# MarToonLi/StableDiffusionEO

Measured on AMD Instinct MI355X. Metric: 512x512 canny2image images/sec (20 DDIM steps); ms per UNet step reported alongside, higher is better.
Workload: dtype f16; 1 GPU; SD1.5 + ControlNet-canny 512x512, batch=1 per GPU (CFG pair fused, N=2), 20 DDIM steps + VAE decode, fp16 storage / fp32 accumulate (BASELINE configs[1]); model_config=sd15, ddim_steps=20, parallelism=dp1 (image index -> rank, RCCL all_gather of final latents), weights=seeded synthetic (no checkpoint in the container)

## Files before the change

stablediffusioneo_amd/csrc/api_ops.hip:

```cpp
#include <stdarg.h>

#include "../../include/sdeo.h"
#include "sdeo_internal.h"
#include "kernels.h"

namespace sdeo {

static thread_local std::string g_last_error;

void set_error(const std::string& msg) { g_last_error = msg; }

int fail(const char* fmt, ...) {
  char buf[1024];
  va_list ap;
  va_start(ap, fmt);
  vsnprintf(buf, sizeof(buf), fmt, ap);
  va_end(ap);
  g_last_error = buf;
  return 1;
}

}

using namespace sdeo;
// ... 253 lines not shown
}

int sdeo_debug_gemm_stats_f16(void* y, int ldy, const void* x, int ldx, const void* w, int ldw, const float* bias, const void* res,
                              int ldres, int m, int n, int k, float* stats, int stats_ld, int* strips_out, void* stream) {
  SDEO_CHECK(stats && strips_out, "gemm_stats: null argument");
  ConvGemm p;
  fill_gemm(p, m, n, k);
  p.x = (const f16*)x; p.w = (const f16*)w; p.bias = bias; p.res = (const f16*)res; p.y = (f16*)y;
  p.ldx = ldx; p.ldw = ldw; p.ldy = ldy; p.ldres = ldres;
  *strips_out = conv_gemm_stats_strips(p);
  if (*strips_out == 0) return 0;
  SDEO_CHECK(*strips_out <= stats_ld, "gemm_stats: %d strips do not fit stats_ld %d", *strips_out, stats_ld);
  p.stats_out = stats; p.stats_ld = stats_ld;
  return conv_gemm(p, S(stream));
}

int sdeo_debug_gemm_res_rows_f16(void* y, int ldy, const void* x, int ldx, const void* w, int ldw, const float* bias, const void* res,
                                 int ldres, int res_rows, int m, int n, int k, float* stats, int stats_ld, int* strips_out, void* workspace,
                                 size_t workspace_bytes, void* stream) {
  ConvGemm p;
  fill_gemm(p, m, n, k);
  p.x = (const f16*)x; p.w = (const f16*)w; p.bias = bias; p.res = (const f16*)res; p.y = (f16*)y;
  p.ldx = ldx; p.ldw = ldw; p.ldy = ldy; p.ldres = ldres; p.res_rows = res_rows;
  p.workspace = (float*)workspace; p.workspace_bytes = workspace_bytes;
  if (stats) {
    SDEO_CHECK(strips_out, "gemm_res_rows: null argument");
    *strips_out = conv_gemm_stats_strips(p);
    SDEO_CHECK(*strips_out <= stats_ld, "gemm_res_rows: %d strips do not fit stats_ld %d", *strips_out, stats_ld);
    if (*strips_out > 0) { p.stats_out = stats; p.stats_ld = stats_ld; }
  }
  return conv_gemm(p, S(stream));
}

int sdeo_debug_gemm_ln_f16(void* y, int ldy, const void* x, int ldx, const void* w_folded, int ldw, const float* ln_s,
                           const float* bias_folded, const float* stats, int stats_ld, int strips, int ln_c, int m, int n, int k, int act, float eps, void* workspace, size_t workspace_bytes, void* stream) {
  ConvGemm p;
  fill_gemm(p, m, n, k);
  p.x = (const f16*)x; p.w = (const f16*)w_folded; p.bias = bias_folded; p.y = (f16*)y;
  p.ldx = ldx; p.ldw = ldw; p.ldy = ldy; p.act = act;
  p.ln_stats = stats; p.ln_s = ln_s; p.ln_strips = strips; p.ln_ld = stats_ld; p.ln_c = ln_c; p.ln_eps = eps;
  p.workspace = (float*)workspace; p.workspace_bytes = workspace_bytes;
  return conv_gemm(p, S(stream));
}

int sdeo_debug_row_stats_f16(float* stats, int stats_ld, const void* x, int ldx, int rows, int c, void* stream) {
  return row_stats(stats, stats_ld, (const f16*)x, ldx, rows, c, S(stream));
}

int sdeo_layernorm_f16(void* y, const void* x, const float* gamma, const float* beta, int rows, int c, float eps,
                       void* stream) {
  return layernorm((f16*)y, c, (const f16*)x, c, gamma, beta, rows, c, eps, S(stream));
}

int sdeo_debug_layernorm_ld_f16(void* y, int ldy, const void* x, int ldx, const float* gamma, const float* beta, int rows, int c,
                                float eps, void* stream) {
  SDEO_CHECK(ldx >= c && ldy >= c, "layernorm_ld: ldx=%d ldy=%d below c=%d", ldx, ldy, c);
  return layernorm((f16*)y, ldy, (const f16*)x, ldx, gamma, beta, rows, c, eps, S(stream));
}

int sdeo_debug_softmax_rows(void* p, int ldp, const float* s, int lds, int rows, int cols, float scale, void* stream) {
  SDEO_CHECK(ldp >= cols && lds >= cols, "softmax_rows: ldp=%d lds=%d below cols=%d", ldp, lds, cols);
  return softmax_rows((f16*)p, ldp, s, lds, rows, cols, scale, S(stream));
}

int sdeo_attention_f16(void* o, int ldo, const void* q, int ldq, const void* k, int ldk, const void* v, int ldv, int b,
                       int heads, int tq, int tk, int tk_stride, int vt_batch_stride, int d, float scale, void* stream) {
// ... 59 lines not shown
```

stablediffusioneo_amd/csrc/conv_gemm.hip:

```cpp
#include <stdlib.h>

#include <array>
#include <map>

#include <type_traits>
#include <utility>

#include "conv_inl.h"

namespace sdeo {

template <int BM, int BN, int STAGES, bool UPS, bool WS, bool W8 = false, int KPB = 1, bool MX = false>
__global__ __launch_bounds__(WS ? 512 : 256) void conv_gemm_dma_kernel(const KP pp) {
  kernarg_warm<sizeof(KP)>();
  KP pl = pp;
  asm volatile("" : "+s"(pl.M), "+s"(pl.N), "+s"(pl.K), "+s"(pl.Hi), "+s"(pl.Wi), "+s"(pl.Cin), "+s"(pl.Wo),
               "+s"(pl.S), "+s"(pl.stride), "+s"(pl.pad), "+s"(pl.HoWo), "+s"(pl.ldx), "+s"(pl.ldw), "+s"(pl.nk),
               "+s"(pl.nk_per_split), "+s"(pl.tiles_m), "+s"(pl.tiles_n), "+s"(pl.n_fastest));
  const KP& p = pl;
  static_assert(!MX || (WS && !W8 && !UPS && KPB == 1), "the block-scaled fp8 path exists for the plain wave-specialised GEMM");
  constexpr int BK = 64, RPP = 32;
  constexpr int WRPP = W8 ? 64 : 32;
  constexpr int XP = BM / RPP, WP = (BN + WRPP - 1) / WRPP, L = XP + WP;
  constexpr int TM = BM / 2, TN = BN / 2, MI = TM / 16, NI = TN / 16;
  constexpr int XBYTES = BM * BK * 2, WBYTES = WP * 4096, STAGE = XBYTES + WBYTES;
  constexpr int PF = STAGES - KPB;
  constexpr int FLY = STAGES - 2 * KPB;
  static_assert(KPB >= 1 && FLY >= 0 && PF >= 1 && STAGES <= 10, "ring depth");

  extern __shared__ __attribute__((aligned(16))) char smem[];

  const int wave_all = __builtin_amdgcn_readfirstlane(threadIdx.x >> 6);
  const bool do_load = !WS || wave_all >= 4;
  const bool do_mma = !WS || wave_all < 4;
  const int tid = threadIdx.x & 255, lane = tid & 63, wave = tid >> 6;
  const int wm = wave & 1, wn = wave >> 1;
  int m0, n0;
  auto set_tile = [&](int t) {
    const int tile = xcd_remap(t, p.tiles_m * p.tiles_n);
    const int tm = p.n_fastest ? tile / p.tiles_n : tile % p.tiles_m;
    const int tn = p.n_fastest ? tile % p.tiles_n : tile / p.tiles_m;
    m0 = tm * BM; n0 = tn * BN;
  };
  set_tile(blockIdx.x);
  const int z = blockIdx.z;
  const int kbeg = z * p.nk_per_split;
  const int kend = min(p.nk, kbeg + p.nk_per_split);
  const int nk = kend - kbeg;

  stamp(p, 0);
  const int chunk = tid & 7, lrow = tid >> 3;
  const int cl = chunk ^ ((lrow >> 1) & 7);
  const char* zero = reinterpret_cast<const char*>(g_zero_page);
  const int wave_u = __builtin_amdgcn_readfirstlane(wave);

  const char* xrow[XP];
  unsigned vmask[XP];
  int pixbase[UPS ? XP : 1], hb[UPS ? XP : 1], wb[UPS ? XP : 1];
  const char* wptr[WP];
  int winc[WP];
  const int tapsteps = p.Cin >> 6;
  int st_c, st_r, st_s;
  auto loader_setup = [&]() {
    st_c = kbeg % tapsteps; st_r = (kbeg / tapsteps) / p.S; st_s = (kbeg / tapsteps) % p.S;
    const int Hv = UPS ? 2 * p.Hi : p.Hi, Wv = UPS ? 2 * p.Wi : p.Wi;
    const int R = p.K / (p.S * p.Cin);
    const bool linear = !UPS && p.K == p.Cin && p.stride == 1 && p.pad == 0;
#pragma unroll
    for (int i = 0; i < XP; ++i) {
      const int m = m0 + lrow + i * RPP;
      const bool mv = m < p.M;
      if (linear) {
        vmask[i] = (mv && !dbg_on(p, 1)) ? 1u : 0u;
        xrow[i] = reinterpret_cast<const char*>(p.x) + ((long)m * p.ldx + cl * 8) * 2;
        continue;
      }
      const int mm = mv ? m : 0;
// ... 291 lines not shown
              reads0(sbn);
            }
          } else {
            reads0(sbn);
            asm volatile("s_waitcnt lgkmcnt(%0)" ::"n"(NI + MI) : "memory");
          }
          __builtin_amdgcn_sched_barrier(0);
          if (!dbg_on(p, 4)) mma_half(wf1, xf1);
          __builtin_amdgcn_sched_barrier(0);
          if (more) reads1(sbn);
          ++ing;
        }
      } else {
        for (int it = 0; it < nk; ++it) {
          if (it % KPB == 0) __builtin_amdgcn_s_barrier();
          if (!dbg_on(p, 4)) compute(it);
        }
      }
    } else {
#pragma unroll
      for (int s = 0; s < PF; ++s)
        if (s < nk) issue(s);
      for (int it = 0; it < nk; ++it) {
        if (it % KPB == 0) {
          retire(it / KPB);
          __builtin_amdgcn_s_barrier();
          refill(it / KPB);
        }
        compute(it);
      }
    }
  }
  KP pe = p;
  pin_epilogue_scalars(pe);
  __builtin_amdgcn_s_barrier();
  stamp(p, 3);
  if (dbg_on(p, 32)) return;
  static_assert(4 * epilogue_scratch_bytes(TN) <= STAGES * STAGE, "epilogue scratch");
  constexpr int SCR = (STAGES * STAGE / 4) & ~15;
  constexpr int NBLK = epilogue_blocks(TN, MI, SCR);
  char* scratch = smem + wave * SCR;
  epilogue<NI, MI, TM, TN, NBLK>(pe, acc, m0, n0, wm, wn, frow, fq, z, bpre, use_bpre, scratch, ln_lds ? lnsm + wm * TM : nullptr);
  if (pe.gn_out) {
    asm volatile("s_waitcnt lgkmcnt(0)" ::: "memory");
    __builtin_amdgcn_s_barrier();
    if (wm == 0) {
      const int bimg = m0 / pe.HoWo;
      gn_partials_finish<TN, 2>(pe, smem + 2 * wn * SCR, SCR, lane, bimg, (m0 - bimg * pe.HoWo) / BM, n0 + wn * TN);
    }
  }
  if (dbg_on(p, 64)) {
    stamp(p, 4);
    asm volatile("s_waitcnt vmcnt(0)" ::: "memory");
    stamp(p, 5);
  }
}

template <int BM, int BN, int BK, bool GENERIC>
__global__ __launch_bounds__(256) void conv_gemm_kernel(const KP pp) {
  kernarg_warm<sizeof(KP)>();
  const KP& p = pp;
  constexpr int CPR = BK / 8;
  constexpr int RPP = 256 / CPR;
  constexpr int XP = BM / RPP;
  constexpr int WP = BN / RPP;
  constexpr int TM = BM / 2, TN = BN / 2;
// ... 196 lines not shown
#pragma unroll
    for (int t = 0; t < 4; ++t) v[t] = gelu_erf_f(v[t]);
  }
  v *= p.scale;
#pragma unroll
  for (int t = 0; t < 4; ++t) v[t] += (float)rv[t];
  if (p.y32) {
    *reinterpret_cast<f32x4*>(p.y32 + (size_t)m * p.ldy + n) = v;
  } else {
    f16x4 o;
#pragma unroll
    for (int t = 0; t < 4; ++t) o[t] = (f16)v[t];
    *reinterpret_cast<f16x4*>(p.y + (size_t)m * p.ldy + n) = o;
  }
}

template <typename K>
static int launch_k(K kernel, int smem, DeviceOnce* attr_done, const KP& kp, int tiles, hipStream_t stream, int threads = 256) {
  if (attr_done->need()) {
    SDEO_HIP(hipFuncSetAttribute(reinterpret_cast<const void*>(kernel), hipFuncAttributeMaxDynamicSharedMemorySize, smem));
    attr_done->mark();
  }
  hipLaunchKernelGGL(kernel, dim3(tiles, 1, kp.splitk), dim3(threads), smem, stream, kp);
  SDEO_HIP(hipGetLastError());
  return 0;
}

template <int BM, int BN, int ST, bool UPS, bool WS, bool W8 = false, int KPB = 1, bool MX = false>
static int launch_dma(const KP& kp, int tiles, hipStream_t stream) {
  static DeviceOnce done;
  constexpr int smem = ST * (W8 ? BM * 128 + (BN + 63) / 64 * 4096 : (BM + BN) * 128) + BM * 8;
  static_assert(smem <= 160 * 1024, "LDS");
  return launch_k(&conv_gemm_dma_kernel<BM, BN, ST, UPS, WS, W8, KPB, MX>, smem, &done, kp, tiles, stream, WS ? 512 : 256);
}

template <int BM, int BN>
static int launch_generic(const KP& kp, int tiles, hipStream_t stream) {
  static DeviceOnce done;
  return launch_k(&conv_gemm_kernel<BM, BN, 32, true>, 2 * (BM + BN) * 64, &done, kp, tiles, stream);
}

template <int BM, int BN, int ST, int CAPS = 0, int KPB = 1>
static constexpr TileCfg dma_tile(const char* name) {
  constexpr bool WS = !(CAPS & CAP_LIGHT);
  TileCfg c{BM, BN, 64, ST, TK_DMA, CAPS | (KPB > 1 ? CAP_GROUPED : 0), KPB, 0, 0, name,
            &launch_dma<BM, BN, ST, false, WS, false, KPB>, &launch_dma<BM, BN, ST, true, WS, false, KPB>, nullptr, nullptr};
  if constexpr ((CAPS & CAP_W8) != 0) c.w8 = &launch_dma<BM, BN, ST, false, true, true>;
  if constexpr ((CAPS & CAP_MX) != 0) c.mx = &launch_dma<BM, BN, ST, false, true, false, 1, true>;
  return c;
}
template <int BM, int BN>
static constexpr TileCfg generic_tile(const char* name) {
  return {BM, BN, 32, 2, TK_GENERIC, 0, 1, 0, 0, name, &launch_generic<BM, BN>, &launch_generic<BM, BN>, nullptr, nullptr};
}
static const TileCfg kTiles[] = {
    dma_tile<128, 128, 3, CAP_MX>("conv_gemm_dma_kernel<128,128,3>"),
    dma_tile<128, 64, 3, CAP_W8 | CAP_MX>("conv_gemm_dma_kernel<128,64,3>"),
    dma_tile<64, 64, 4, CAP_W8>("conv_gemm_dma_kernel<64,64,4>"),
    generic_tile<128, 64>("conv_gemm_kernel<128,64,32,true>"),
    generic_tile<64, 64>("conv_gemm_kernel<64,64,32,true>"),
    dma_tile<256, 128, 3>("conv_gemm_dma_kernel<256,128,3>"),
    dma_tile<64, 160, 3, CAP_W8 | CAP_MX>("conv_gemm_dma_kernel<64,160,3>"),
    dma_tile<128, 160, 3>("conv_gemm_dma_kernel<128,160,3>"),
    dma_tile<256, 160, 3>("conv_gemm_dma_kernel<256,160,3>"),
    dma_tile<32, 160, 4, CAP_W8>("conv_gemm_dma_kernel<32,160,4>"),
    dma_tile<64, 160, 5>("conv_gemm_dma_kernel<64,160,5>"),
// ... 256 lines not shown
    const size_t need = (size_t)pl.splitk * p.M * p.N * sizeof(float);
    SDEO_CHECK(p.workspace && p.workspace_bytes >= need, "conv_gemm: split-K workspace too small (%zu < %zu)",
               p.workspace_bytes, need);
  }
  if (kTiles[pl.tile].kind == TK_HALO) SDEO_CHECK(halo_ok(p, kTiles[pl.tile]), "conv_gemm: halo plan on an ineligible problem");
  return 0;
}

static int dispatch(const Plan& pl, int ups, bool w8, const KP& kp, hipStream_t stream) {
  if (pl.tile < 0 || pl.tile >= kTileCount) return fail("conv_gemm: bad tile %d", pl.tile);
  const TileCfg& c = kTiles[pl.tile];
  const TileLaunch launch = kp.mx_sx ? c.mx : w8 ? c.w8 : ups ? c.ups : c.plain;
  if (!launch) return fail("conv_gemm: tile %d has no %s instantiation", pl.tile, kp.mx_sx ? "block-scaled fp8" : w8 ? "fp8-weight" : "folded-upsample");
  if (int rc = launch(kp, pl.tiles_m * pl.tiles_n, stream)) return rc;
  if (pl.splitk > 1) {
    const int64_t n = (int64_t)kp.M * (kp.N / 4);
    hipLaunchKernelGGL(splitk_reduce_kernel, dim3((unsigned)cdiv64(n, 256)), dim3(256), 0, stream, kp);
    SDEO_HIP(hipGetLastError());
  }
  return 0;
}

int conv_gemm(const ConvGemm& p0, hipStream_t stream) {
  if (p0.mx_sx)
    SDEO_CHECK(p0.K % 128 == 0 && p0.ldx % 16 == 0 && p0.ldw % 16 == 0 && p0.K == p0.Cin, "conv_gemm: block-scaled fp8 GEMM needs K %% 128 == 0 (K=%d, ldx=%d, ldw=%d)", p0.K, p0.ldx, p0.ldw);
  const ConvGemm p = mx_view(p0);
  Plan pl;
  KP kp{};
  if (int rc = prepare(p, pl, kp)) return rc;
  g_last_tile = pl.tile; g_last_splitk = pl.splitk;
  return dispatch(pl, p.ups, p.wscale != nullptr, kp, stream);
}

int conv_gemm_tile_info(int tile, int* kind, int* bm, int* bn, int* stages, int* caps, const char** name) {
  if (tile < 0 || tile >= kTileCount) return 1;
  const TileCfg& c = kTiles[tile];
  *kind = c.kind; *bm = c.bm; *bn = c.bn; *stages = c.stages; *caps = c.caps; *name = c.name;
  return 0;
}

int conv_gemm_read_stamps(unsigned long long* out, int n) {
  SDEO_HIP(hipDeviceSynchronize());
  SDEO_HIP(hipMemcpyFromSymbol(out, HIP_SYMBOL(g_stamps), sizeof(unsigned long long) * (size_t)(n < kStampWGs * kStampSlots ? n : kStampWGs * kStampSlots)));
  return 0;
}

void conv_gemm_set_tuned(const int key[10], int tile, int splitk) {
  ShapeKey k;
  for (int i = 0; i < 10; ++i) k[i] = key[i];
  if (tile >= 0 && tile < kTileCount && kTiles[tile].kind != TK_GENERIC && splitk >= 1) g_tuned[k] = {tile, splitk};
}

std::string conv_gemm_tuned_json() {
  std::string out = "[";
  char buf[256];
  bool first = true;
  for (auto& kv : g_tuned) {
    snprintf(buf, sizeof(buf), "%s[%d,%d,%d,%d,%d,%d,%d,%d,%d,%d,%d,%d]", first ? "" : ",", kv.first[0], kv.first[1], kv.first[2],
             kv.first[3], kv.first[4], kv.first[5], kv.first[6], kv.first[7], kv.first[8], kv.first[9], kv.second.first,
             kv.second.second);
    out += buf;
    first = false;
  }
  return out + "]";
}

// ... 64 lines not shown
```

stablediffusioneo_amd/csrc/conv_inl.h:

```cpp
#pragma once
#include <utility>

#include "kernels.h"

namespace sdeo {

struct KP {
  const f16* x;
  const f16* w;
  f16* y;
  float* y32;
  const float* bias;
  const float* bias2;
  const f16* res;
  float* ws;
  int M, N, K;
  int Hi, Wi, Cin, Ho, Wo, S, stride, pad, ups;
  int HoWo;
  int ldx, ldw, ldy, ldres, ld_bias2;
  int res_rows;
  int act, bias_per_row;
  float scale;
  int nk, nk_per_split, splitk;
  int tiles_m, tiles_n;
  int dbg;
  int n_fastest;
  int coalesce;
  const float* ln_stats;
  const float* ln_s;
  int ln_strips, ln_ld;
  float ln_invc, ln_eps;
  const float* wscale;
  float* stats_out;
  int stats_ld;
  float* gn_out;
  int gn_cpg, gn_slots, gn_groups;
  const unsigned char* mx_sx;
  const unsigned char* mx_sw;
  int mx_ldsx, mx_ldsw;
};

#ifdef SDEO_DEBUG_KERNELS
__device__ __forceinline__ bool dbg_on(const KP& p, int bit) { return (p.dbg & bit) != 0; }
#else
__device__ __forceinline__ constexpr bool dbg_on(const KP&, int) { return false; }
#endif

constexpr int kStampWGs = 4096, kStampSlots = 16;
static __device__ unsigned long long g_stamps[kStampWGs * kStampSlots];
__device__ __forceinline__ void stamp_cycles(const KP& p, int slot) {
  if (dbg_on(p, 64) && threadIdx.x == 0) {
    const int wg = blockIdx.x + gridDim.x * blockIdx.z;
    if (wg < kStampWGs) g_stamps[wg * kStampSlots + slot] = __builtin_amdgcn_s_memtime();
  }
}
__device__ __forceinline__ void stamp(const KP& p, int slot) {
  if (dbg_on(p, 64) && threadIdx.x == 0) {
    const int wg = blockIdx.x + gridDim.x * blockIdx.z;
    if (wg < kStampWGs) g_stamps[wg * kStampSlots + slot] = __builtin_amdgcn_s_memrealtime();
  }
}

static __device__ __attribute__((aligned(256))) const unsigned int g_zero_page[64] = {0};

template <int BK>
__device__ __forceinline__ int swz_chunk(int row, int chunk) {
  if (BK == 64) return chunk ^ ((row >> 1) & 7);
  return chunk ^ (((row >> 3) & 1) * 3);
}

constexpr int epilogue_scratch_bytes(int tn) { return 16 * (tn * 4 + 16) + 32 * tn; }

__device__ __forceinline__ unsigned long long pin_u64(unsigned long long v) {
  unsigned lo = __builtin_amdgcn_readfirstlane((unsigned)v), hi = __builtin_amdgcn_readfirstlane((unsigned)(v >> 32));
// ... 472 lines not shown
```

stablediffusioneo_amd/csrc/handle_common.h:

```cpp
#pragma once
#include <stdlib.h>

#include <algorithm>
#include <functional>
#include <string>
#include <unordered_map>
#include <vector>

#include "arena.h"
#include "kernels.h"

namespace sdeo {

enum WKind { W_CONV, W_LINEAR, W_VEC, W_GEGLU_W, W_GEGLU_B };
struct WEntry {
  std::string name;
  int64_t dims[4];
  int ndim;
  WKind kind;
  size_t off;
  int ipad;
  bool loaded;
};

struct WeightStore {
  std::vector<WEntry> entries;
  std::unordered_map<std::string, int> index;
  size_t size = 0;
  char* slab = nullptr;
  size_t slab_bytes = 0;
  float* stage = nullptr;
  size_t stage_bytes = 0;

  size_t take(size_t bytes) {
    const size_t off = align_up(size, 256);
    size = off + bytes;
    return off;
  }
  void add(const std::string& name, WKind kind, std::initializer_list<int64_t> dims, size_t off, int ipad = 0) {
    WEntry w{name, {1, 1, 1, 1}, (int)dims.size(), kind, off, ipad, false};
    int i = 0;
    for (auto d : dims) w.dims[i++] = d;
    index[name] = (int)entries.size();
// ... 125 lines not shown
      for (; i < aggs.size(); ++i) if (aggs[i].first == r.key) break;
      if (i == aggs.size()) aggs.push_back({r.key, Agg()});
      aggs[i].second.n += 1; aggs[i].second.ms += ms; aggs[i].second.flops += r.flops; aggs[i].second.bytes += r.bytes;
    }
    recs.clear();
    report = "[";
    char buf[768];
    for (size_t i = 0; i < aggs.size(); ++i) {
      snprintf(buf, sizeof(buf), "%s{\"kernel\": \"%s\", \"launches\": %ld, \"total_ms\": %.6f, \"flops\": %.6e, \"bytes\": %.6e}",
               i ? ", " : "", aggs[i].first.c_str(), aggs[i].second.n, aggs[i].second.ms, aggs[i].second.flops, aggs[i].second.bytes);
      report += buf;
    }
    report += "]";
    return report.c_str();
  }
};

struct WorkspaceRef { float* const* p; const size_t* bytes; };

static inline Op conv_gemm_op(const ConvGemm& p0, WorkspaceRef ws, size_t* max_ws, bool tagged = false, int flop_k = 0,
                              std::function<void(ConvGemm&)> late = nullptr) {
  *max_ws = std::max(*max_ws, conv_gemm_workspace_bytes(p0));
  return Op([p = p0, ws, late](hipStream_t s) mutable {
    p.workspace = *ws.p;
    p.workspace_bytes = *ws.bytes;
    if (late) late(p);
    return conv_gemm(p, s);
  }, conv_gemm_kernel_name(p0), 2.0 * p0.M * p0.N * (double)(flop_k ? flop_k : p0.K),
     2.0 * ((double)p0.M * p0.Cin + (double)p0.N * p0.K + (double)p0.M * p0.N),
     !tagged ? std::string() : "M" + std::to_string(p0.M) + " N" + std::to_string(p0.N) + " K" + std::to_string(p0.K) + " R" +
         std::to_string(p0.R) + " s" + std::to_string(p0.stride) + " u" + std::to_string(p0.ups));
}

static inline int run_program(const Program& p, hipStream_t s, Profiler* prof = nullptr) {
  if (!prof || !prof->on) {
    for (auto& op : p)
      if (int rc = op(s)) return rc;
    return 0;
  }
  for (auto& op : p)
    if (int rc = prof->record(op, s)) return rc;
  return 0;
}

}
```

stablediffusioneo_amd/csrc/kernels.h:

```cpp
#pragma once
#include "common.h"

namespace sdeo {

struct ConvGemm {
  const f16* x = nullptr;
  const f16* w = nullptr;
  f16* y = nullptr;
  float* y32 = nullptr;
  const float* bias = nullptr;
  const float* bias2 = nullptr;
  const f16* res = nullptr;
  float* workspace = nullptr;
  size_t workspace_bytes = 0;
  int M = 0, N = 0, K = 0;
  int B = 1, Hi = 1, Wi = 1, Cin = 0;
  int Ho = 1, Wo = 1, R = 1, S = 1, stride = 1, pad = 0;
  int pad_after = -1;
  int ups = 0;
  int ldx = 0, ldw = 0, ldy = 0, ldres = 0, ld_bias2 = 0;
  int act = 0;
  int bias_per_row = 0;
  float scale = 1.0f;
  int force_tile = -1;
  int force_splitk = 0;
  const float* ln_stats = nullptr;
  const float* ln_s = nullptr;
  int ln_strips = 0, ln_ld = 0;
  int ln_c = 0;
  float ln_eps = 1e-5f;
  const float* wscale = nullptr;
  float* stats_out = nullptr;
  int stats_ld = 0;
  float* gn_out = nullptr;
  int gn_cpg = 0, gn_slots = 0, gn_groups = 0;
  const uint8_t* mx_sx = nullptr;
  const uint8_t* mx_sw = nullptr;
  int mx_ldsx = 0, mx_ldsw = 0;
  int res_rows = 0;
  int plan_B = 0;
};
int conv_gemm(const ConvGemm& p, hipStream_t stream);
inline int conv_pad_after(const ConvGemm& p) { return p.pad_after < 0 ? p.pad : p.pad_after; }
int conv_gemm_gn_slots(const ConvGemm& p, int cpg);
bool conv_gemm_plan_is_halo(const ConvGemm& p);
int conv_gemm_stats_strips(const ConvGemm& p);
int conv_gemm_read_stamps(unsigned long long* out, int n);
int conv_halo_read_stamps(unsigned long long* out, int n);
size_t conv_gemm_workspace_bytes(const ConvGemm& p);
int conv_gemm_plan_splitk(const ConvGemm& p);
void conv_gemm_query_plan(const ConvGemm& p, int key[10], int* tile, int* splitk);
void conv_gemm_last_plan(int* tile, int* splitk);
int conv_gemm_tile_info(int tile, int* kind, int* bm, int* bn, int* stages, int* caps, const char** name);
const char* conv_gemm_kernel_name(const ConvGemm& p);
void conv_gemm_debug_force(int tile, int splitk);
void conv_gemm_debug_force_order(int order);
int conv_gemm_autotune(const ConvGemm& p, hipStream_t stream);
size_t conv_gemm_autotune_workspace_bytes(const ConvGemm& p);
void conv_gemm_set_tuned(const int key[10], int tile, int splitk);
std::string conv_gemm_tuned_json();

int gn_chunks(int HW);
int groupnorm_nhwc(f16* y, int ldy, const f16* x, int ldx, const float* gamma, const float* beta, int B, int HW, int C,
                   int groups, float eps, int with_silu, float* partials, hipStream_t stream);

struct GnArgs {
  f16* y; const f16* x; const float* gamma; const float* beta; float* partials;
  int ldy, ldx, B, HW, C, groups;
  float eps;
  int with_silu;
  const float* ext_partials = nullptr;
  int ext_nsc = 0;
};
bool groupnorm_is_single_launch(const GnArgs& a);
int gn_fused_threads(const GnArgs& a);
int groupnorm_nhwc(const GnArgs& a, hipStream_t stream);
// ... 68 lines not shown
```

stablediffusioneo_amd/csrc/net.hip:

```cpp
#include <functional>
#include <memory>
#include <unordered_map>
#include <vector>

#include "../../include/sdeo.h"
#include "handle_common.h"
#include "net_plan.h"

using namespace sdeo;

namespace {

static inline int round8(int c) { return (c + 7) / 8 * 8; }

struct FoldJob { size_t w_out, s_out, b_out, w_in; std::string gamma, beta, bias; int rows, C; };
struct ComposeJob { size_t w_out, b_out; std::string wp, bp, w2, b2; int C; };
struct QRegion { size_t off; int rows, cols; size_t q_off, s_off; };

struct Builder;

struct Fp8State {
  std::vector<QRegion> qregions;
  std::unordered_map<size_t, int> qindex;
  int weight_bits = 16;
// ... 824 lines not shown
  for (size_t i = 0; i < e->cplan.in.size(); ++i) {
    if (i == 0) {
      Builder::CO o; o.res = &c.hint_feat; o.gn_next = true;
      hcur = b.conv(hcur, ns + e->cplan.in[0][0].name, e->cfg.model_channels, 3, 1, 0, o);
    } else if (i == 1) {
      hcur = build_shared_prefix(c, ns, e->cplan.in[i], hcur, 1, sp);
    } else {
      hcur = run_blocks(c, ns, e->cplan.in[i], hcur, false, 1, nullptr);
    }
    e->cn_h[i] = hcur;
    zero_conv(hcur, ns + "zero_convs." + std::to_string(i) + ".0", e->cplan.in_ch[i], &e->ctrl[i]);
  }
  T m = run_blocks(c, ns, e->cplan.mid, hcur, false, 1, nullptr);
  e->cn_h[c.nctrl - 1] = m;
  zero_conv(m, ns + "middle_block_out.0", e->cplan.in_ch.back(), &e->ctrl[c.nctrl - 1]);
  splice(c, e->prog[P_CN_SH], p_cn, sp);
}

static void build_control_io(BuildCtx& c) {
  Engine* e = c.b.e;
  e->ctrl_elems.clear();
  for (int i = 0; i < c.nctrl; ++i) {
    const T& t = e->ctrl[i];
    e->ctrl_elems.push_back((size_t)t.n * t.c * t.h * t.w);
    if (c.b.dry) continue;
    float* o = e->out_ctrl[i]; const f16* in = t.p; const int N = c.N, ld = t.ld, Cc = t.c, HW = t.h * t.w;
    e->prog[P_CN_EXPORT].push_back([=](hipStream_t s) { return nhwc_f16_to_nchw_f32(o, in, ld, N, Cc, HW, 1.0f, s); });
    const float* ci = e->in_ctrl[i]; f16* co = t.p;
    e->prog[P_CTRL_IMPORT].push_back([=](hipStream_t s) { return nchw_f32_to_nhwc_f16(co, ld, ci, N, Cc, HW, 1.0f, s); });
  }
}

enum DecoderMode { D_NOCTRL, D_ADD, D_FUSED };
static void build_unet_decoder(BuildCtx& c, DecoderMode mode, std::vector<T> hs, T cat, T view) {
  Builder& b = c.b; Engine* e = b.e;
  const std::string ns = NS_UNET;
  int ci = c.nctrl - 1;
  if (mode == D_ADD) {
    f16* yp = view.p; const int ld = view.ld, rows = view.rows(), Cc = view.c;
    const f16* cp = e->ctrl[ci].p; const int ldc = e->ctrl[ci].ld; const float* sc = &e->scales[ci];
    b.push([=](hipStream_t s) { return add_scaled(yp, ld, yp, ld, cp, ldc, *sc, rows, Cc, s); });
  } else if (mode == D_FUSED) {
    Builder::CO zo; zo.out = &view; zo.res = &view; zo.scale_host = &e->eff_scales[ci];
    b.conv(e->cn_h[ci], std::string(NS_CN) + "middle_block_out.0", view.c, 1, 1, 0, zo);
  }
  --ci;
  for (size_t oi = 0; oi < e->uplan.out.size(); ++oi) {
    T skip = hs.back();
    hs.pop_back();
    const int c_h = cat.c - skip.c;
    if (mode == D_FUSED) {
      const T half = cat.view(c_h, skip.c);
      Builder::CO zo; zo.out = &half; zo.res = &skip; zo.scale_host = &e->eff_scales[ci];
      b.conv(e->cn_h[ci], std::string(NS_CN) + "zero_convs." + std::to_string(ci) + ".0", skip.c, 1, 1, 0, zo);
    } else {
      f16* yp = cat.p + c_h; const int ld = cat.ld, rows = cat.rows(), Cc = skip.c;
      const f16* ap = skip.p; const int lda = skip.ld;
      const f16* cp = mode == D_ADD ? e->ctrl[ci].p : nullptr; const int ldc = mode == D_ADD ? e->ctrl[ci].ld : 0;
      const float* sc = &e->scales[ci]; const int* om = &e->only_mid;
      b.push([=](hipStream_t s) { return add_scaled(yp, ld, ap, lda, (*om) ? nullptr : cp, ldc, *sc, rows, Cc, s); });
    }
    --ci;
    b.release(skip);
    const std::vector<Blk>& blocks = e->uplan.out[oi];
    if (oi + 1 < e->uplan.out.size()) {
      const T& nskip = hs.back();
      const int c_hn = blocks.back().cout;
      const int up = blocks.back().kind == B_UP ? 2 : 1;
      T ncat = b.alloc(cat.n, cat.h * up, cat.w * up, c_hn + nskip.c);
      const T nview = ncat.view(0, c_hn);
      run_blocks(c, ns, blocks, cat, true, 0, &nview);
      cat = ncat;
    } else {
      T y = run_blocks(c, ns, blocks, cat, true, 0, nullptr);
      Builder::CO oo; oo.cout_store = 4 * ((e->cfg.out_channels + 3) / 4);
      oo.out = &e->eps16;
      b.gn_conv(y, ns + "out.0", 1e-5f, 1, ns + "out.2", e->cfg.out_channels, oo);
      b.release(y);
    }
  }
}

static void build_unet(BuildCtx& c, bool with_ctrl) {
  Builder& b = c.b; Engine* e = b.e;
  b.prog = &e->prog[with_ctrl ? P_UNET_ENC : P_UNET_NOCTRL];
  const std::string ns = NS_UNET;
  std::vector<T> hs;
  T hcur = e->x0;
  Splice sp;
  for (size_t i = 0; i < e->uplan.in.size(); ++i) {
    hcur = (i == 1 && with_ctrl) ? build_shared_prefix(c, ns, e->uplan.in[i], hcur, 0, sp) : run_blocks(c, ns, e->uplan.in[i], hcur, false, 0, nullptr);
    hs.push_back(hcur);
  }
  const int c_mid = e->uplan.mid.back().cout;
  const T cat0 = b.alloc(hcur.n, hcur.h, hcur.w, c_mid + hcur.c), view0 = cat0.view(0, c_mid);
  run_blocks(c, ns, e->uplan.mid, hcur, false, 0, &view0);
  if (!with_ctrl) return build_unet_decoder(c, D_NOCTRL, hs, cat0, view0);
  splice(c, e->prog[P_UNET_ENC_SH], e->prog[P_UNET_ENC], sp);
  Arena& arena = *b.lane->arena;
  const Arena after_encoder = arena;
  b.prog = &e->prog[P_UNET_DEC];
  build_unet_decoder(c, D_ADD, hs, cat0, view0);
  const size_t peak_add = arena.peak;
  arena = after_encoder;
  arena.peak = std::max(arena.peak, peak_add);
  b.prog = &e->prog[P_UNET_DEC_FUSED];
  build_unet_decoder(c, D_FUSED, hs, cat0, view0);
// ... 611 lines not shown
```

stablediffusioneo_amd/csrc/sdeo_internal.h:

```cpp
#ifndef SDEO_INTERNAL_H
#define SDEO_INTERNAL_H

#include <stdint.h>

#ifdef __cplusplus
extern "C" {
#endif

void sdeo_debug_force_gemm_plan(int tile, int splitk);
void sdeo_debug_force_gemm_order(int order);
const char* sdeo_debug_conv2d_kernel_name(int n, int h, int w, int cin, int cout, int ksize, int stride, int upsample2x);
const char* sdeo_debug_attention_kernel_name(int B, int H, int Tq, int Tk, int d, int causal);
int sdeo_debug_conv2d_plan(int n, int h, int w, int cin, int cout, int ksize, int stride, int upsample2x, int act, int fp8, int* key10,
                           int* tile, int* splitk);
int sdeo_debug_gemm_plan(int m, int n, int k, int act, int fp8, int* key10, int* tile, int* splitk);
void sdeo_debug_last_gemm_plan(int* tile, int* splitk);
int sdeo_debug_tile_info(int tile, int* kind, int* bm, int* bn, int* stages, int* caps, const char** name);
int sdeo_debug_read_stamps(int which, unsigned long long* out, int n);
int sdeo_debug_silu(void* y, const void* x, int64_t n, void* stream);

int sdeo_debug_groupnorm_path(int n, int hw, int c, int groups);
int sdeo_debug_groupnorm_ld_f16(void* y, int ldy, const void* x, int ldx, const float* gamma, const float* beta, int n, int hw, int c,
                                int groups, float eps, int with_silu, void* workspace, void* stream);
int sdeo_debug_layernorm_ld_f16(void* y, int ldy, const void* x, int ldx, const float* gamma, const float* beta, int rows, int c,
                                float eps, void* stream);
int sdeo_debug_softmax_rows(void* p, int ldp, const float* s, int lds, int rows, int cols, float scale, void* stream);

int sdeo_debug_fold_layernorm(void* w_out, float* s_out, float* b_out, const void* w, const float* gamma, const float* beta,
                              const float* bias, int rows, int c, void* stream);
int sdeo_debug_compose_proj(void* w_out, float* b_out, const void* wp, const float* bp, const void* w2, const float* b2, int c, int k2,
                            void* stream);
int sdeo_debug_gemm_stats_f16(void* y, int ldy, const void* x, int ldx, const void* w, int ldw, const float* bias, const void* res,
                              int ldres, int m, int n, int k, float* stats, int stats_ld, int* strips_out, void* stream);
int sdeo_debug_gemm_ln_f16(void* y, int ldy, const void* x, int ldx, const void* w_folded, int ldw, const float* ln_s,
                           const float* bias_folded, const float* stats, int stats_ld, int strips, int ln_c, int m, int n, int k, int act, float eps, void* workspace, size_t workspace_bytes, void* stream);
int sdeo_debug_row_stats_f16(float* stats, int stats_ld, const void* x, int ldx, int rows, int c, void* stream);
int sdeo_debug_conv2d_gn_f16(void* ynorm, void* y, const void* x, const void* w_krsc, const float* bias, const void* res, int n, int h,
                             int w, int cin, int cout, int ksize, int stride, int upsample2x, const float* gamma, const float* beta,
                             int groups, float eps, int with_silu, float* partials, size_t partial_floats, int* slots, void* stream);

int sdeo_debug_gemm_res_rows_f16(void* y, int ldy, const void* x, int ldx, const void* w, int ldw, const float* bias, const void* res,
                                 int ldres, int res_rows, int m, int n, int k, float* stats, int stats_ld, int* strips_out, void* workspace,
                                 size_t workspace_bytes, void* stream);
int sdeo_debug_attention_qb_f16(void* o, int ldo, const void* q, int ldq, const void* k, int ldk, const void* v, int ldv, int b,
                                int q_batches, int heads, int tq, int tk, int tk_stride, int v_batch_stride, int d, float scale, void* stream);

int sdeo_debug_quantize_mx(void* q_out, void* scales_out, const void* x, int rows, int cols, void* stream);
int sdeo_debug_gemm_mx_f16(void* y, int ldy, const void* xq, const void* xs, const void* wq, const void* ws, const float* bias, const void* res,
// ... 17 lines not shown
```

stablediffusioneo_amd/ops.py:

```python
from __future__ import annotations

import ctypes as C

import torch

from . import _lib
from ._lib import check, cur_stream, ptr


def _need_cuda(*ts):
    for t in ts:
        if t is not None and not t.is_cuda:
            raise _lib.SdeoError("HIP ops need device tensors (no CPU fallback)")


def _ws(nbytes, device):
    return torch.empty(max(int(nbytes), 16), dtype=torch.uint8, device=device)


def _nhwc_ld(t, what):
    n, h, w, _ = t.shape
    ld = t.stride(2)
    assert t.dtype == torch.float16 and t.stride(3) == 1 and (h == 1 or t.stride(1) == w * ld) and (n == 1 or t.stride(0) == h * w * ld), \
        f"groupnorm: {what} must be fp16 NHWC with unit channel stride and densely stacked pixels (shape {tuple(t.shape)}, strides {t.stride()})"
# ... 132 lines not shown
    hv, wv = (2 * h, 2 * w) if upsample2x else (h, w)
    pad = k // 2
    ho = (hv + 2 * pad - k) // stride + 1
    wo = (wv + 2 * pad - k) // stride + 1
    y = torch.empty((n, ho, wo, cout), dtype=torch.float16, device=x.device)
    yn = torch.empty_like(y)
    pf = n * (ho * wo) * groups * 2 // 16 + n * groups * 2 + 1024
    part = torch.empty(pf, dtype=torch.float32, device=x.device)
    slots = C.c_int(0)
    check(lib.sdeo_debug_conv2d_gn_f16(ptr(yn), ptr(y), ptr(x), ptr(w_krsc), ptr(bias), ptr(res), n, h, w, cin, cout, k, stride,
                                       int(upsample2x), ptr(gamma), ptr(beta), groups, eps, int(swish), ptr(part), pf, C.byref(slots),
                                       cur_stream()), "conv2d_gn")
    if slots.value == 0:
        return None
    return y, yn, slots.value


def gemm(x, w, bias=None, res=None, act=0, scale=1.0, out_f32=False, bias_per_row=False, w8=None, out=None):
    lib = _lib.load()
    _need_cuda(x, w)
    m, k = x.shape
    n, k2 = w.shape
    assert k == k2 and x.stride(1) == 1 and w.stride(1) == 1
    y = _out(out, (m, n), torch.float32 if out_f32 else torch.float16, x.device)
    nb = lib.sdeo_gemm_workspace_bytes(m, n, k)
    ws = _ws(nb if w8 is None else max(nb, 64 << 20), x.device)
    _arm_fp8(lib, w8)
    check(lib.sdeo_gemm_f16(ptr(y), n, ptr(x), x.stride(0), ptr(w), w.stride(0), ptr(bias), ptr(res),
                            res.stride(0) if res is not None else 0, m, n, k, act, scale, int(out_f32), int(bias_per_row), ptr(ws),
                            ws.numel(), cur_stream()), "gemm")
    return y


def fold_layernorm(w, gamma, beta, bias=None):
    lib = _lib.load()
    _need_cuda(w, gamma, beta)
    rows, c = w.shape
    assert w.dtype == torch.float16 and w.is_contiguous()
    wo = torch.empty_like(w)
    s = torch.empty((rows,), dtype=torch.float32, device=w.device)
    b = torch.empty((rows,), dtype=torch.float32, device=w.device)
    check(lib.sdeo_debug_fold_layernorm(ptr(wo), ptr(s), ptr(b), ptr(w), ptr(gamma), ptr(beta), ptr(bias), rows, c, cur_stream()),
          "fold_layernorm")
    return wo, s, b


def compose_proj(wp, bp, w2, b2):
    lib = _lib.load()
    _need_cuda(wp, bp, w2, b2)
    c, k2 = w2.shape
    assert wp.shape == (c, c) and wp.dtype == torch.float16 and w2.dtype == torch.float16 and wp.is_contiguous() and w2.is_contiguous()
    wo = torch.empty((c, k2 + c), dtype=torch.float16, device=wp.device)
    bo = torch.empty((c,), dtype=torch.float32, device=wp.device)
    check(lib.sdeo_debug_compose_proj(ptr(wo), ptr(bo), ptr(wp), ptr(bp), ptr(w2), ptr(b2), c, k2, cur_stream()), "compose_proj")
    return wo, bo


def gemm_with_row_stats(x, w, bias=None, res=None):
    lib = _lib.load()
    _need_cuda(x, w)
    m, k = x.shape
    n = w.shape[0]
    y = torch.empty((m, n), dtype=torch.float16, device=x.device)
    ld = max(1, (n + 31) // 32)
    stats = torch.zeros((m, ld, 2), dtype=torch.float32, device=x.device)
    strips = C.c_int(0)
# ... 253 lines not shown
```

Before: 8.342 images/s.

## Batch ControlNet zero-convs into one grouped multi-problem GEMM launch

Adds a grouped GEMM variant of the DMA conv kernel. Each workgroup looks up its problem from a device-resident prefix table and loads that problem's kernel parameters from constant memory. In fused-decoder mode the UNet decoder now issues every ControlNet zero-conv (middle block plus each skip) as a single launch on a fixed 128x64 tile, with each output written into the concat buffers with the skip residual added. The goal is to remove a dozen or so small, poorly occupied kernel launches. The trade-off is a tile chosen for all problems rather than one tuned per problem, and the concat buffers for every stage are allocated up front.

```diff
diff --git a/stablediffusioneo_amd/csrc/api_ops.hip b/stablediffusioneo_amd/csrc/api_ops.hip
--- a/stablediffusioneo_amd/csrc/api_ops.hip
+++ b/stablediffusioneo_amd/csrc/api_ops.hip
@@ -309,6 +309,33 @@
   return conv_gemm(p, S(stream));
 }
 
+int sdeo_debug_gemm_multi_f16(int count, const int* tile, const int* splitk, const int* m, const int* n, const int* k, void* const* y,
+                              const int* ldy, const void* const* x, const int* ldx, const void* const* w, const int* ldw,
+                              const void* const* bias, const void* const* res, const int* ldres, const float* scale, void* stream) {
+  SDEO_CHECK(count >= 1 && tile && splitk && m && n && k && y && ldy && x && ldx && w && ldw && scale, "gemm_multi: null argument");
+  std::vector<ConvGemm> ps((size_t)count);
+  for (int i = 0; i < count; ++i) {
+    ConvGemm& p = ps[i];
+    fill_gemm(p, m[i], n[i], k[i]);
+    p.x = (const f16*)x[i]; p.w = (const f16*)w[i]; p.y = (f16*)y[i];
+    p.bias = bias ? (const float*)bias[i] : nullptr;
+    p.res = res ? (const f16*)res[i] : nullptr;
+    p.ldx = ldx[i]; p.ldw = ldw[i]; p.ldy = ldy[i]; p.ldres = (res && res[i] && ldres) ? ldres[i] : 0;
+    p.scale = scale[i];
+    p.force_tile = tile[i]; p.force_splitk = splitk[i];
+  }
+  ConvGemmMultiPlan pl;
+  if (int rc = conv_gemm_multi_plan(ps, tile[0], &pl)) return rc;
+  void* tab = nullptr;
+  SDEO_HIP(hipMalloc(&tab, pl.table.size()));
+  int rc = 0;
+  if (hipMemcpy(tab, pl.table.data(), pl.table.size(), hipMemcpyHostToDevice) != hipSuccess) rc = fail("gemm_multi: cannot write the problem table");
+  if (!rc) rc = conv_gemm_multi_launch(pl, tab, nullptr, S(stream));
+  if (!rc && hipStreamSynchronize(S(stream)) != hipSuccess) rc = fail("gemm_multi: the launch failed");
+  (void)hipFree(tab);
+  return rc;
+}
+
 int sdeo_debug_gemm_ln_f16(void* y, int ldy, const void* x, int ldx, const void* w_folded, int ldw, const float* ln_s,
                            const float* bias_folded, const float* stats, int stats_ld, int strips, int ln_c, int m, int n, int k, int act, float eps, void* workspace, size_t workspace_bytes, void* stream) {
   ConvGemm p;
diff --git a/stablediffusioneo_amd/csrc/conv_gemm.hip b/stablediffusioneo_amd/csrc/conv_gemm.hip
--- a/stablediffusioneo_amd/csrc/conv_gemm.hip
+++ b/stablediffusioneo_amd/csrc/conv_gemm.hip
@@ -10,10 +10,32 @@
 
 namespace sdeo {
 
-template <int BM, int BN, int STAGES, bool UPS, bool WS, bool W8 = false, int KPB = 1, bool MX = false>
-__global__ __launch_bounds__(WS ? 512 : 256) void conv_gemm_dma_kernel(const KP pp) {
-  kernarg_warm<sizeof(KP)>();
-  KP pl = pp;
+template <int BM, int BN, int STAGES, bool UPS, bool WS, bool W8 = false, int KPB = 1, bool MX = false, bool MULTI = false>
+__global__ __launch_bounds__(WS ? 512 : 256) void conv_gemm_dma_kernel(const std::conditional_t<MULTI, MPArgs, KP> pp) {
+  kernarg_warm<sizeof(pp)>();
+  static_assert(!MULTI || (!W8 && !MX), "multi-problem launches stream fp16 weights");
+  KP pl;
+  int wg = blockIdx.x;
+  [[maybe_unused]] int mp_prob = 0;
+  if constexpr (MULTI) {
+    int pre[kMultiMax];
+#pragma unroll
+    for (int i = 0; i < kMultiMax; ++i) pre[i] = mp_prefix(pp.tab, i);
+    int prob = 0, first = 0;
+#pragma unroll
+    for (int i = 0; i < kMultiMax - 1; ++i) {
+      const bool past = (int)blockIdx.x >= pre[i];
+      prob += past ? 1 : 0;
+      first = past ? pre[i] : first;
+    }
+    mp_prob = __builtin_amdgcn_readfirstlane(min(prob, pp.count - 1));
+    wg = __builtin_amdgcn_readfirstlane((int)blockIdx.x - first);
+    pl = mp_block(pp.tab, mp_prob);
+    pl.scale = pp.scale[mp_prob];
+    mp_globalize(pl);
+  } else {
+    pl = pp;
+  }
   asm volatile("" : "+s"(pl.M), "+s"(pl.N), "+s"(pl.K), "+s"(pl.Hi), "+s"(pl.Wi), "+s"(pl.Cin), "+s"(pl.Wo),
                "+s"(pl.S), "+s"(pl.stride), "+s"(pl.pad), "+s"(pl.HoWo), "+s"(pl.ldx), "+s"(pl.ldw), "+s"(pl.nk),
                "+s"(pl.nk_per_split), "+s"(pl.tiles_m), "+s"(pl.tiles_n), "+s"(pl.n_fastest));
@@ -42,7 +64,7 @@
     const int tn = p.n_fastest ? tile % p.tiles_n : tile / p.tiles_m;
     m0 = tm * BM; n0 = tn * BN;
   };
-  set_tile(blockIdx.x);
+  set_tile(wg);
   const int z = blockIdx.z;
   const int kbeg = z * p.nk_per_split;
   const int kend = min(p.nk, kbeg + p.nk_per_split);
@@ -400,6 +422,7 @@
     }
   }
   KP pe = p;
+  if constexpr (MULTI) { pe = mp_block(pp.tab, mp_prob); pe.scale = pp.scale[mp_prob]; }
   pin_epilogue_scalars(pe);
   __builtin_amdgcn_s_barrier();
   stamp(p, 3);
@@ -662,6 +685,22 @@
   constexpr int smem = ST * (W8 ? BM * 128 + (BN + 63) / 64 * 4096 : (BM + BN) * 128) + BM * 8;
   static_assert(smem <= 160 * 1024, "LDS");
   return launch_k(&conv_gemm_dma_kernel<BM, BN, ST, UPS, WS, W8, KPB, MX>, smem, &done, kp, tiles, stream, WS ? 512 : 256);
+}
+
+typedef int (*MultiLaunch)(const MPArgs& a, int tiles, hipStream_t stream);
+template <int BM, int BN, int ST, bool WS>
+static int launch_dma_multi(const MPArgs& a, int tiles, hipStream_t stream) {
+  static DeviceOnce done;
+  constexpr int smem = ST * (BM + BN) * 128 + BM * 8;
+  static_assert(smem <= 160 * 1024, "LDS");
+  auto kernel = &conv_gemm_dma_kernel<BM, BN, ST, false, WS, false, 1, false, true>;
+  if (done.need()) {
+    SDEO_HIP(hipFuncSetAttribute(reinterpret_cast<const void*>(kernel), hipFuncAttributeMaxDynamicSharedMemorySize, smem));
+    done.mark();
+  }
+  hipLaunchKernelGGL(kernel, dim3(tiles, 1, 1), dim3(WS ? 512 : 256), smem, stream, a);
+  SDEO_HIP(hipGetLastError());
+  return 0;
 }
 
 template <int BM, int BN>
@@ -984,6 +1023,68 @@
   return dispatch(pl, p.ups, p.wscale != nullptr, kp, stream);
 }
 
+struct MultiTile { int tile, bm, bn, stages; bool light; MultiLaunch launch; const char* name; };
+static const MultiTile kMultiTiles[] = {
+    {2, 64, 64, 4, false, &launch_dma_multi<64, 64, 4, true>, "conv_gemm_dma_kernel<64,64,4> multi"},
+    {6, 64, 160, 3, false, &launch_dma_multi<64, 160, 3, true>, "conv_gemm_dma_kernel<64,160,3> multi"},
+    {26, 128, 64, 2, true, &launch_dma_multi<128, 64, 2, false>, "conv_gemm_dma_kernel<128,64,2> multi"},
+};
+static const MultiTile* multi_tile(int tile) {
+  for (const MultiTile& m : kMultiTiles) {
+    const TileCfg& c = kTiles[m.tile];
+    if (m.tile == tile && c.kind == TK_DMA && c.bm == m.bm && c.bn == m.bn && c.stages == m.stages && c.kpb == 1 &&
+        ((c.caps & CAP_LIGHT) != 0) == m.light)
+      return &m;
+  }
+  return nullptr;
+}
+
+int conv_gemm_multi_plan(const std::vector<ConvGemm>& ps, int tile, ConvGemmMultiPlan* out) {
+  *out = ConvGemmMultiPlan{};
+  SDEO_CHECK(!ps.empty() && (int)ps.size() <= kMultiMax, "conv_gemm_multi: %d problems in one launch (1..%d)", (int)ps.size(), kMultiMax);
+  for (const ConvGemm& p : ps) {
+    if (tile < 0) tile = p.force_tile;
+    SDEO_CHECK(p.force_tile < 0 || p.force_tile == tile, "conv_gemm_multi: mixed tiles (%d and %d): one tile serves all problems of a launch", tile, p.force_tile);
+    SDEO_CHECK(p.force_splitk <= 1, "conv_gemm_multi: a split-K plan (factor %d) cannot be part of a multi-problem launch", p.force_splitk);
+  }
+  const MultiTile* mt = multi_tile(tile);
+  SDEO_CHECK(mt, "conv_gemm_multi: tile %d has no multi-problem instantiation", tile);
+  MPTable tab{};
+  int total = 0;
+  for (size_t i = 0; i < ps.size(); ++i) {
+    ConvGemm p = ps[i];
+    SDEO_CHECK(!p.mx_sx && !p.wscale, "conv_gemm_multi: problem %d: fp16 weights only", (int)i);
+    SDEO_CHECK(!p.gn_out && !p.stats_out && !p.ln_stats, "conv_gemm_multi: problem %d: no GroupNorm-partial, row-statistics or LayerNorm-fold epilogue", (int)i);
+    SDEO_CHECK(p.act != 3 && !p.ups && p.plan_B == 0, "conv_gemm_multi: problem %d: no GEGLU pair, folded upsample or batch-prefix plan", (int)i);
+    SDEO_CHECK(is_fast(p), "conv_gemm_multi: problem %d: Cin=%d must be a multiple of 64", (int)i, p.Cin);
+    p.force_tile = tile; p.force_splitk = 1;
+    Plan pl;
+    if (int rc = prepare(p, pl, tab.kp[i])) return rc;
+    SDEO_CHECK(pl.tile == tile && pl.splitk == 1, "conv_gemm_multi: problem %d cannot run unsplit on tile %d", (int)i, tile);
+    total += pl.tiles_m * pl.tiles_n;
+    tab.prefix[i] = total;
+    out->scale[i] = p.scale;
+    out->flops += 2.0 * p.M * p.N * (double)p.K;
+    out->bytes += 2.0 * ((double)p.M * p.Cin + (double)p.N * p.K + (double)p.M * p.N);
+  }
+  for (int i = (int)ps.size(); i < kMultiMax; ++i) tab.prefix[i] = 0x7fffffff;
+  out->tile = tile; out->count = (int)ps.size(); out->tiles = total; out->name = mt->name;
+  out->table.assign(reinterpret_cast<const char*>(&tab), reinterpret_cast<const char*>(&tab) + sizeof(tab));
+  return 0;
+}
+
+int conv_gemm_multi_launch(const ConvGemmMultiPlan& pl, const void* table_dev, const float* scales, hipStream_t stream) {
+  const MultiTile* mt = multi_tile(pl.tile);
+  SDEO_CHECK(mt && pl.count >= 1 && pl.count <= kMultiMax && pl.tiles > 0 && pl.table.size() == sizeof(MPTable), "conv_gemm_multi: launch of an unplanned table");
+  SDEO_CHECK(table_dev && (reinterpret_cast<uintptr_t>(table_dev) & 15) == 0, "conv_gemm_multi: the device table must be 16-byte aligned");
+  MPArgs a{};
+  a.tab = static_cast<const MPTable*>(table_dev);
+  a.count = pl.count;
+  for (int i = 0; i < pl.count; ++i) a.scale[i] = scales ? scales[i] : pl.scale[i];
+  g_last_tile = pl.tile; g_last_splitk = 1;
+  return mt->launch(a, pl.tiles, stream);
+}
+
 int conv_gemm_tile_info(int tile, int* kind, int* bm, int* bn, int* stages, int* caps, const char** name) {
   if (tile < 0 || tile >= kTileCount) return 1;
   const TileCfg& c = kTiles[tile];
diff --git a/stablediffusioneo_amd/csrc/conv_inl.h b/stablediffusioneo_amd/csrc/conv_inl.h
--- a/stablediffusioneo_amd/csrc/conv_inl.h
+++ b/stablediffusioneo_amd/csrc/conv_inl.h
@@ -1,4 +1,5 @@
 #pragma once
+#include <type_traits>
 #include <utility>
 
 #include "kernels.h"
@@ -40,6 +41,37 @@
   int mx_ldsx, mx_ldsw;
 };
 
+struct MPTable {
+  int prefix[kMultiMax];
+  KP kp[kMultiMax];
+};
+struct MPArgs {
+  const MPTable* tab;
+  int count;
+  float scale[kMultiMax];
+};
+__device__ __forceinline__ int mp_prefix(const MPTable* tab, int i) {
+#if defined(__HIP_DEVICE_COMPILE__)
+  return ((const __attribute__((address_space(4))) MPTable*)tab)->prefix[i];
+#else
+  return tab->prefix[i];
+#endif
+}
+__device__ __forceinline__ KP mp_block(const MPTable* tab, int prob) {
+#if defined(__HIP_DEVICE_COMPILE__)
+  return ((const __attribute__((address_space(4))) MPTable*)tab)->kp[prob];
+#else
+  return tab->kp[prob];
+#endif
+}
+__device__ __forceinline__ void mp_globalize(KP& q) {
+#define SDEO_GLOBAL_PTR(f) q.f = (decltype(q.f))(__attribute__((address_space(1))) std::remove_pointer_t<decltype(q.f)>*)q.f;
+  SDEO_GLOBAL_PTR(x) SDEO_GLOBAL_PTR(w) SDEO_GLOBAL_PTR(y) SDEO_GLOBAL_PTR(y32) SDEO_GLOBAL_PTR(bias) SDEO_GLOBAL_PTR(bias2)
+  SDEO_GLOBAL_PTR(res) SDEO_GLOBAL_PTR(ws) SDEO_GLOBAL_PTR(ln_stats) SDEO_GLOBAL_PTR(ln_s) SDEO_GLOBAL_PTR(wscale)
+  SDEO_GLOBAL_PTR(stats_out) SDEO_GLOBAL_PTR(gn_out) SDEO_GLOBAL_PTR(mx_sx) SDEO_GLOBAL_PTR(mx_sw)
+#undef SDEO_GLOBAL_PTR
+}
+
 #ifdef SDEO_DEBUG_KERNELS
 __device__ __forceinline__ bool dbg_on(const KP& p, int bit) { return (p.dbg & bit) != 0; }
 #else
diff --git a/stablediffusioneo_amd/csrc/handle_common.h b/stablediffusioneo_amd/csrc/handle_common.h
--- a/stablediffusioneo_amd/csrc/handle_common.h
+++ b/stablediffusioneo_amd/csrc/handle_common.h
@@ -3,12 +3,16 @@
 
 #include <algorithm>
 #include <functional>
+#include <memory>
+#include <set>
 #include <string>
 #include <unordered_map>
 #include <vector>
 
 #include "arena.h"
 #include "kernels.h"
+
+extern "C" const char* sdeo_last_error(void);
 
 namespace sdeo {
 
@@ -200,6 +204,31 @@
          std::to_string(p0.R) + " s" + std::to_string(p0.stride) + " u" + std::to_string(p0.ups));
 }
 
+static inline Op conv_gemm_multi_op(const std::vector<ConvGemm>& ps, int tile, std::vector<const float*> scale_host = {}) {
+  static std::set<std::string> keys;
+  auto pl = std::make_shared<ConvGemmMultiPlan>();
+  std::shared_ptr<void> dev;
+  std::string err;
+  if (conv_gemm_multi_plan(ps, tile, pl.get())) {
+    err = sdeo_last_error();
+  } else {
+    void* d = nullptr;
+    if (hipMalloc(&d, pl->table.size()) != hipSuccess || hipMemcpy(d, pl->table.data(), pl->table.size(), hipMemcpyHostToDevice) != hipSuccess) {
+      (void)hipGetLastError();
+      err = "conv_gemm_multi: cannot place the problem table in device memory";
+    }
+    dev.reset(d, [](void* q) { if (q) (void)hipFree(q); });
+  }
+  scale_host.resize(ps.size(), nullptr);
+  const char* key = keys.insert(std::string(err.empty() ? pl->name : "conv_gemm multi") + " x" + std::to_string(ps.size())).first->c_str();
+  return Op([pl, dev, err, scale_host](hipStream_t s) {
+    if (!err.empty()) return fail("%s", err.c_str());
+    float sc[kMultiMax];
+    for (int i = 0; i < pl->count; ++i) sc[i] = scale_host[i] ? *scale_host[i] : pl->scale[i];
+    return conv_gemm_multi_launch(*pl, dev.get(), sc, s);
+  }, key, pl->flops, pl->bytes, "tiles" + std::to_string(pl->tiles));
+}
+
 static inline int run_program(const Program& p, hipStream_t s, Profiler* prof = nullptr) {
   if (!prof || !prof->on) {
     for (auto& op : p)
diff --git a/stablediffusioneo_amd/csrc/kernels.h b/stablediffusioneo_amd/csrc/kernels.h
--- a/stablediffusioneo_amd/csrc/kernels.h
+++ b/stablediffusioneo_amd/csrc/kernels.h
@@ -1,4 +1,6 @@
 #pragma once
+#include <vector>
+
 #include "common.h"
 
 namespace sdeo {
@@ -42,6 +44,16 @@
 };
 int conv_gemm(const ConvGemm& p, hipStream_t stream);
 inline int conv_pad_after(const ConvGemm& p) { return p.pad_after < 0 ? p.pad : p.pad_after; }
+constexpr int kMultiMax = 16;
+struct ConvGemmMultiPlan {
+  int tile = -1, count = 0, tiles = 0;
+  std::vector<char> table;
+  float scale[kMultiMax] = {};
+  double flops = 0, bytes = 0;
+  const char* name = "";
+};
+int conv_gemm_multi_plan(const std::vector<ConvGemm>& ps, int tile, ConvGemmMultiPlan* out);
+int conv_gemm_multi_launch(const ConvGemmMultiPlan& pl, const void* table_dev, const float* scales, hipStream_t stream);
 int conv_gemm_gn_slots(const ConvGemm& p, int cpg);
 bool conv_gemm_plan_is_halo(const ConvGemm& p);
 int conv_gemm_stats_strips(const ConvGemm& p);
diff --git a/stablediffusioneo_amd/csrc/net.hip b/stablediffusioneo_amd/csrc/net.hip
--- a/stablediffusioneo_amd/csrc/net.hip
+++ b/stablediffusioneo_amd/csrc/net.hip
@@ -880,9 +880,19 @@
 }
 
 enum DecoderMode { D_NOCTRL, D_ADD, D_FUSED };
+static const int kZeroConvTile = 26;
+static bool zero_convs_as_one(const BuildCtx& c) {
+  const Engine* e = c.b.e;
+  if (c.nctrl > kMultiMax || e->fp8.act_bits == 8 || e->uplan.out.size() + 1 != (size_t)c.nctrl) return false;
+  for (int i = 0; i < c.nctrl; ++i)
+    if (e->cn_h[i].c % 64) return false;
+  return true;
+}
+static void build_unet_decoder_multi(BuildCtx& c, std::vector<T> hs, T cat0, T view0);
 static void build_unet_decoder(BuildCtx& c, DecoderMode mode, std::vector<T> hs, T cat, T view) {
   Builder& b = c.b; Engine* e = b.e;
   const std::string ns = NS_UNET;
+  if (mode == D_FUSED && zero_convs_as_one(c)) return build_unet_decoder_multi(c, hs, cat, view);
   int ci = c.nctrl - 1;
   if (mode == D_ADD) {
     f16* yp = view.p; const int ld = view.ld, rows = view.rows(), Cc = view.c;
@@ -921,6 +931,54 @@
       cat = ncat;
     } else {
       T y = run_blocks(c, ns, blocks, cat, true, 0, nullptr);
+      Builder::CO oo; oo.cout_store = 4 * ((e->cfg.out_channels + 3) / 4);
+      oo.out = &e->eps16;
+      b.gn_conv(y, ns + "out.0", 1e-5f, 1, ns + "out.2", e->cfg.out_channels, oo);
+      b.release(y);
+    }
+  }
+}
+
+static void build_unet_decoder_multi(BuildCtx& c, std::vector<T> hs, T cat0, T view0) {
+  Builder& b = c.b; Engine* e = b.e;
+  const std::string ns = NS_UNET;
+  const size_t stages = e->uplan.out.size(), nh = hs.size();
+  std::vector<T> cats{cat0};
+  for (size_t oi = 0; oi + 1 < stages; ++oi) {
+    const std::vector<Blk>& blocks = e->uplan.out[oi];
+    const T& prev = cats.back();
+    const int up = blocks.back().kind == B_UP ? 2 : 1;
+    cats.push_back(b.alloc(prev.n, prev.h * up, prev.w * up, blocks.back().cout + hs[nh - 2 - oi].c));
+  }
+  std::vector<ConvGemm> zc;
+  std::vector<const float*> zs;
+  auto zero_conv = [&](int ci, const std::string& name, const T& out, const T& res) {
+    const T& x = e->cn_h[ci];
+    const WEntry* w = b.W(name + ".weight");
+    if (w && w->ipad != x.c && b.err.empty()) b.err = "conv " + name + ": input has " + std::to_string(x.c) + " channels, weight expects " + std::to_string(w->ipad);
+    ConvGemm p;
+    p.x = x.p; p.w = b.wptr(name + ".weight"); p.bias = b.vptr(name + ".bias"); p.y = out.p; p.res = res.p;
+    p.B = x.n; p.Hi = p.Ho = x.h; p.Wi = p.Wo = x.w; p.Cin = x.c;
+    p.M = x.rows(); p.N = out.c; p.K = x.c;
+    p.ldx = x.ld; p.ldw = p.K; p.ldy = out.ld; p.ldres = res.ld;
+    zc.push_back(p);
+    zs.push_back(&e->eff_scales[ci]);
+  };
+  int ci = c.nctrl - 1;
+  zero_conv(ci--, std::string(NS_CN) + "middle_block_out.0", view0, view0);
+  for (size_t oi = 0; oi < stages; ++oi, --ci) {
+    const T& skip = hs[nh - 1 - oi];
+    zero_conv(ci, std::string(NS_CN) + "zero_convs." + std::to_string(ci) + ".0", cats[oi].view(cats[oi].c - skip.c, skip.c), skip);
+  }
+  if (!b.dry) b.prog->push_back(conv_gemm_multi_op(zc, kZeroConvTile, zs));
+  for (T& skip : hs) b.release(skip);
+  for (size_t oi = 0; oi < stages; ++oi) {
+    const std::vector<Blk>& blocks = e->uplan.out[oi];
+    if (oi + 1 < stages) {
+      const T nview = cats[oi + 1].view(0, blocks.back().cout);
+      run_blocks(c, ns, blocks, cats[oi], true, 0, &nview);
+    } else {
+      T y = run_blocks(c, ns, blocks, cats[oi], true, 0, nullptr);
       Builder::CO oo; oo.cout_store = 4 * ((e->cfg.out_channels + 3) / 4);
       oo.out = &e->eps16;
       b.gn_conv(y, ns + "out.0", 1e-5f, 1, ns + "out.2", e->cfg.out_channels, oo);
diff --git a/stablediffusioneo_amd/csrc/sdeo_internal.h b/stablediffusioneo_amd/csrc/sdeo_internal.h
--- a/stablediffusioneo_amd/csrc/sdeo_internal.h
+++ b/stablediffusioneo_amd/csrc/sdeo_internal.h
@@ -14,6 +14,9 @@
 int sdeo_debug_conv2d_plan(int n, int h, int w, int cin, int cout, int ksize, int stride, int upsample2x, int act, int fp8, int* key10,
                            int* tile, int* splitk);
 int sdeo_debug_gemm_plan(int m, int n, int k, int act, int fp8, int* key10, int* tile, int* splitk);
+int sdeo_debug_gemm_multi_f16(int count, const int* tile, const int* splitk, const int* m, const int* n, const int* k, void* const* y,
+                              const int* ldy, const void* const* x, const int* ldx, const void* const* w, const int* ldw,
+                              const void* const* bias, const void* const* res, const int* ldres, const float* scale, void* stream);
 void sdeo_debug_last_gemm_plan(int* tile, int* splitk);
 int sdeo_debug_tile_info(int tile, int* kind, int* bm, int* bn, int* stages, int* caps, const char** name);
 int sdeo_debug_read_stamps(int which, unsigned long long* out, int n);
diff --git a/stablediffusioneo_amd/ops.py b/stablediffusioneo_amd/ops.py
--- a/stablediffusioneo_amd/ops.py
+++ b/stablediffusioneo_amd/ops.py
@@ -188,6 +188,32 @@
     return y
 
 
+def gemm_multi(problems, tile, tiles=None, splitk=None):
+    lib = _lib.load()
+    cnt = len(problems)
+    outs, keep = [], []
+    arr_i = lambda vals: (C.c_int * cnt)(*[int(v) for v in vals])
+    arr_p = lambda ts: (C.c_void_p * cnt)(*[t.data_ptr() if t is not None else None for t in ts])
+    for p in problems:
+        x, w = p["x"], p["w"]
+        _need_cuda(x, w)
+        assert x.shape[1] == w.shape[1] and x.stride(1) == 1 and w.stride(1) == 1
+        y = p.get("out")
+        if y is None:
+            y = torch.empty((x.shape[0], w.shape[0]), dtype=torch.float16, device=x.device)
+        assert y.shape == (x.shape[0], w.shape[0]) and y.stride(1) == 1 and y.dtype == torch.float16
+        outs.append(y)
+    res = [p.get("res") for p in problems]
+    check(lib.sdeo_debug_gemm_multi_f16(
+        cnt, arr_i(tiles if tiles is not None else [tile] * cnt), arr_i(splitk if splitk is not None else [1] * cnt),
+        arr_i(p["x"].shape[0] for p in problems), arr_i(p["w"].shape[0] for p in problems), arr_i(p["x"].shape[1] for p in problems),
+        arr_p(outs), arr_i(y.stride(0) for y in outs), arr_p([p["x"] for p in problems]), arr_i(p["x"].stride(0) for p in problems),
+        arr_p([p["w"] for p in problems]), arr_i(p["w"].stride(0) for p in problems), arr_p([p.get("bias") for p in problems]),
+        arr_p(res), arr_i(r.stride(0) if r is not None else 0 for r in res),
+        (C.c_float * cnt)(*[float(p.get("scale", 1.0)) for p in problems]), cur_stream()), "gemm_multi")
+    return outs
+
+
 def fold_layernorm(w, gamma, beta, bias=None):
     lib = _lib.load()
     _need_cuda(w, gamma, beta)
```

Measured after the change: 8.445 images/s, median of 6. 1.2% higher.
